# Dhole/collaborative_filtering

Measured on AMD Instinct MI355X. Metric: user-subgraph eigendecomps/sec + predicted ratings/sec, 1M users avg deg 100, higher is better.
Workload: dtype f32 (eigen) / f64 (predict)

## Files before the change

### collaborative_filtering_amd/_native.py

```python
from __future__ import annotations

import ctypes
import os
from ctypes import POINTER, c_char_p, c_double, c_float, c_int, c_int32, c_uint32, c_uint64, c_void_p

_HERE = os.path.dirname(os.path.abspath(__file__))
LIB_PATH = os.environ.get("CF_MI355X_LIB") or os.path.join(_HERE, "libcf_mi355x.so")
HOST_LIB_PATH = os.path.join(_HERE, "libcf_host.so")

CF_OK = 0
CF_EINVAL = -1
CF_ERANGE = -4
CF_ESTATE = -5
CF_KNN_SCORE_SUM = 0
CF_KNN_SCORE_MEAN = 1
CF_NMF_OBSERVED = 0
CF_NMF_GRID = 1
CF_NMF_EPS = 1e-16
CF_BPR_TRIES = 8
CF_SVD_MAX_NV = 256
CF_ALS_MAX_D = 64
CF_TOPN_MAX_N = 1024
CF_SIGS_OWN = 0
CF_SIGS_COMPAT = 1
CF_MAX_K = 192
CF_SPILL_MAX_K = 5000
CF_EIGEN_TRIDIAG = 0
CF_EIGEN_JACOBI = 1
CF_GRAPH_DENSE = 0
CF_GRAPH_CSR = 1
CF_FILTER_CHEBY = 0
CF_FILTER_BINOMIAL = 1

SIGNATURES = {
    "cf_version": (c_int, []),
    "cf_device_count": (c_int, []),
    "cf_create": (c_int, [c_int, POINTER(c_void_p)]),
    "cf_destroy": (None, [c_void_p]),
    "cf_release_workspaces": (c_int, [c_void_p]),
    "cf_last_error": (c_char_p, [c_void_p]),
    "cf_set_jacobi": (c_int, [c_void_p, c_float, c_int]),
    "cf_set_eigen_refine": (c_int, [c_void_p, c_int, c_float, c_float]),
    "cf_set_eigen_split": (c_int, [c_void_p, c_int]),
    "cf_set_eigen_lanes": (c_int, [c_void_p, c_int]),
    "cf_debug_eigen_geometry": (c_int, [c_int, c_int, POINTER(c_int), POINTER(c_int), POINTER(c_int), POINTER(c_int),
                                        POINTER(c_int)]),
    "cf_set_pred_pack": (c_int, [c_void_p, c_int]),
    "cf_debug_split_schedule": (c_int, [c_int, c_int, POINTER(c_int), POINTER(c_int), POINTER(c_int), POINTER(c_int)]),
    "cf_set_step_masks": (c_int, [c_void_p, c_int]),
    "cf_set_local_wlim": (c_int, [c_void_p, c_int]),
    "cf_debug_predict_nmax": (c_int, [c_int]),
    "cf_set_knn2_topk": (c_int, [c_void_p, c_uint32]),
    "cf_set_eigen_method": (c_int, [c_void_p, c_int]),
    "cf_debug_stats": (c_int, [c_void_p, c_int, c_void_p]),
    "cf_eigen_bucket_timing": (c_int, [c_void_p, c_int, c_void_p]),
    "cf_eigen_bucket_timing_split": (c_int, [c_void_p, c_int, c_void_p, c_void_p]),
    "cf_debug_phases": (c_int, [c_void_p, c_int, c_void_p]),
    "cf_debug_spill": (c_int, [c_void_p, c_int, c_void_p]),
    "cf_debug_tri": (c_int, [c_void_p, c_int, c_void_p]),
    "cf_item_graph_upload": (c_int, [c_void_p, c_uint32, c_void_p, c_void_p, c_void_p]),
    "cf_item_graph_upload_dense": (c_int, [c_void_p, c_uint32, c_void_p, c_int]),
    "cf_item_graph_device": (c_void_p, [c_void_p, POINTER(c_uint32)]),
    "cf_set_graph_layout": (c_int, [c_void_p, c_int]),
    "cf_graph_info": (c_int, [c_void_p, c_void_p, c_void_p, c_void_p]),
    "cf_item_cosine_edges": (c_int, [c_void_p, c_uint32, c_uint32, c_void_p, c_void_p, c_void_p, c_float, c_int, c_int,
                                     c_void_p, c_void_p, c_void_p, c_uint64, c_void_p]),
    "cf_plan_create": (c_int, [c_void_p, c_uint32, c_void_p, POINTER(c_void_p)]),
    "cf_plan_destroy": (None, [c_void_p]),
    "cf_evec_slots": (c_uint64, [c_uint32]),
    "cf_evec_offsets": (c_uint64, [c_uint32, c_void_p, c_void_p]),
    "cf_eigen_batch": (c_int, [c_void_p, c_uint32, c_void_p, c_void_p, c_void_p, c_void_p, c_void_p,
                               c_void_p, c_void_p]),
    "cf_eigen_run": (c_int, [c_void_p, c_void_p, c_void_p, c_void_p, c_void_p, c_void_p, c_void_p,
                             c_void_p, c_void_p, c_void_p]),
    "cf_predict_precomp": (c_int, [c_void_p, c_uint32, c_void_p, c_void_p, c_void_p, c_void_p, c_void_p,
                                   c_void_p, c_void_p, c_void_p, c_uint64, c_int, c_void_p, c_void_p,
                                   c_void_p]),
    "cf_predict_precomp_sel": (c_int, [c_void_p, c_uint32, c_void_p, c_void_p, c_void_p, c_void_p, c_void_p,
                                       c_void_p, c_void_p, c_void_p, c_uint64, c_int, c_void_p, c_void_p,
                                       c_void_p, c_void_p]),
# ... 238 lines not shown
```

### collaborative_filtering_amd/api.py

```python
from __future__ import annotations

from ctypes import byref, c_double, c_float, c_int, c_uint32, c_void_p
from dataclasses import dataclass

import numpy as np

from . import _native
from ._native import CF_ERANGE, CF_FILTER_BINOMIAL, CF_FILTER_CHEBY, CF_SIGS_COMPAT, CF_SIGS_OWN, NativeError, ptr


def _check(lib, ctx, rc, what):
    if rc != _native.CF_OK:
        msg = lib.cf_last_error(ctx)
        raise NativeError(f"{what} failed ({rc}): {msg.decode() if msg else ''}")


def evec_offsets(item_off: np.ndarray) -> tuple[np.ndarray, int]:
    k = np.diff(item_off.astype(np.int64))
    slots = k * np.maximum(k, 2)
    off = np.zeros(len(k), dtype=np.uint64)
    if len(k):
        off[1:] = np.cumsum(slots)[:-1]
    return off, int(slots.sum())

# ... 312 lines not shown
    def __enter__(self):
        return self

    def __exit__(self, *exc):
        self.close()

    def __del__(self):
        try:
            self.close()
        except Exception:
            pass

    def _chk(self, rc, what):
        _check(self.lib, self.h, rc, what)

    def set_eigen_method(self, method: str = "jacobi"):
        code = {"tridiag": _native.CF_EIGEN_TRIDIAG, "jacobi": _native.CF_EIGEN_JACOBI}[method]
        self._chk(self.lib.cf_set_eigen_method(self.h, code), "cf_set_eigen_method")

    def set_jacobi(self, tol_scale: float = 1.0, max_sweeps: int = 30):
        self._chk(self.lib.cf_set_jacobi(self.h, tol_scale, max_sweeps), "cf_set_jacobi")

    def set_eigen_refine(self, enable: bool = True, stop_rel: float = 1e-3, delta: float = 1e-2):
        self._chk(self.lib.cf_set_eigen_refine(self.h, int(enable), stop_rel, delta), "cf_set_eigen_refine")

    def set_eigen_split(self, enable=True):
        self._chk(self.lib.cf_set_eigen_split(self.h, int(enable)), "cf_set_eigen_split")

    def set_eigen_lanes(self, lanes=0):
        self._chk(self.lib.cf_set_eigen_lanes(self.h, int(lanes)), "cf_set_eigen_lanes")

    def set_pred_pack(self, mode=1):
        self._chk(self.lib.cf_set_pred_pack(self.h, int(mode)), "cf_set_pred_pack")

    def set_local_wlim(self, bisect: bool = True):
        self._chk(self.lib.cf_set_local_wlim(self.h, int(bisect)), "cf_set_local_wlim")

    def set_step_masks(self, enable: bool = True):
        self._chk(self.lib.cf_set_step_masks(self.h, int(enable)), "cf_set_step_masks")

    def debug_stats(self, enable: bool = True, read: bool = False):
        out = np.zeros(8, dtype=np.uint64) if read else None
        self._chk(self.lib.cf_debug_stats(self.h, int(enable), ptr(out)), "cf_debug_stats")
        if read:
            n = max(int(out[1]), 1)
            return {"sweeps_mean": int(out[0]) / n, "users": int(out[1]), "sweeps_max": int(out[2]),
                    "capped": int(out[3]), "assembly_cyc_per_user": int(out[4]) / n,
                    "jacobi_cyc_per_user": int(out[5]) / n, "epilogue_cyc_per_user": int(out[6]) / n,
                    "jacobi_cyc_per_step": int(out[5]) / max(int(out[7]), 1)}
        return None

    def eigen_bucket_timing(self, enable: bool = True, read: bool = False, sweeps: bool = False):
        out = np.zeros(13, dtype=np.float32) if read else None
        sw = np.zeros(13, dtype=np.float32) if read else None
        self._chk(self.lib.cf_eigen_bucket_timing_split(self.h, int(enable), ptr(out), ptr(sw)),
                  "cf_eigen_bucket_timing_split")
        return (out, sw) if sweeps else out

    def debug_spill(self, enable: bool = True, read: bool = False):
        out = np.zeros(8, dtype=np.uint64) if read else None
        self._chk(self.lib.cf_debug_spill(self.h, int(enable), ptr(out)), "cf_debug_spill")
        if read:
            n = max(int(out[0]), 1)
            names = ["assembly", "tridiag", "accumulate", "ql", "ql_gen"]
            r = {f"{nm}_cyc_per_user": int(out[i + 1]) / n for i, nm in enumerate(names)}
            r.update(users=int(out[0]), ql_iters_per_user=int(out[6]) / n, output_cyc_per_user=int(out[7]) / n)
# ... 962 lines not shown
```

### collaborative_filtering_amd/csrc/cf_internal.h

```cpp
#pragma once

#include <hip/hip_runtime.h>

#include <algorithm>
#include <cstdint>
#include <string>
#include <vector>

#include "cf_abi.h"

struct GraphRow {
    const float* dense;
    const uint32_t* col;
    const float* w;
    uint32_t len;
    __device__ __forceinline__ float operator[](uint32_t b) const {
        if (dense) return dense[b];
        uint32_t lo = 0, hi = len;
        while (lo < hi) {
            const uint32_t mid = (lo + hi) >> 1;
            if (col[mid] < b) lo = mid + 1;
            else hi = mid;
        }
        return (lo < len && col[lo] == b) ? w[lo] : 0.0f;
// ... 71 lines not shown
    size_t tri_bytes = 0;
    int eigen_method = CF_EIGEN_JACOBI;
    bool tri_debug = false;
    hipEvent_t knn_ev[3] = {nullptr, nullptr, nullptr};
    int knn_path = 0;
    unsigned int* d_knn_acc = nullptr;
    void* d_knn_part = nullptr;
    size_t knn_part_bytes = 0;
    uint32_t knn_chunk_users = 0;
    uint32_t knn2_topk = 0;
    int knn_chunks = 0;
    void* d_prep = nullptr;
    size_t prep_bytes = 0;
    hipEvent_t prep_ev[2] = {nullptr, nullptr};
    static constexpr int kAuxStreams = 2;
    hipStream_t aux_stream[kAuxStreams] = {};
    hipEvent_t aux_event[kAuxStreams + 1] = {};
    static constexpr int kBucketRuns = 16;
    bool bucket_timing = false;
    hipEvent_t bucket_ev[kBucketRuns][13][3] = {};
    bool bucket_recorded[kBucketRuns][13] = {};
    bool bucket_mid[kBucketRuns][13] = {};
    hipEvent_t split_mid_ev = nullptr;
    bool split_mid_recorded = false;
    int bucket_run = 0;
    hipStream_t step_stream[2] = {};
    hipEvent_t step_bucket_ev[16] = {};
    hipEvent_t step_sync_ev[4] = {};
    hipEvent_t step_time_ev[3] = {};
    uint32_t* d_split_sched[13] = {};
    int eigen_lanes = -1;
    int eigen_split = -1;
    int pred_pack = -1;
    int split_finish = -1;
    float filter_ms = 0.0f;
    uint64_t filter_nnz = 0;
    void* d_als = nullptr;
    size_t als_bytes = 0;
    float sgd_reduce_ms[2] = {0.0f, 0.0f};
    float svdpp_reduce_ms[3] = {0.0f, 0.0f, 0.0f};
    float bpr_ms[6] = {0.0f, 0.0f, 0.0f, 0.0f, 0.0f, 0.0f};
    uint32_t topn_block = 0;
    uint64_t* d_knn_in_off = nullptr;
    uint32_t* d_knn_in_m = nullptr;
    float* d_knn_in_w = nullptr;
    uint32_t* d_knn_in_cnt = nullptr;
    double knn_in_wmin = 0.0;
    uint64_t knn_in_gen = ~0ull;
    int knn_topn_wgs = -1;
    double* d_ease_B = nullptr;
    uint32_t ease_n = 0;
    float ease_ms[3] = {0.0f, 0.0f, 0.0f};
};

void cf_ease_free(cf_ctx* ctx);

void cf_knn_in_free(cf_ctx* ctx);

struct PanelSource {
    virtual ~PanelSource() = default;
    virtual bool valid() const = 0;
    virtual size_t workspace(uint32_t ub) const = 0;
    virtual int upload(cf_ctx* ctx, void* ws, uint32_t ub, hipStream_t st, float* score_ms) = 0;
    virtual int fill(cf_ctx* ctx, hipStream_t st, const uint32_t* d_sel, uint32_t b0, uint32_t nb, uint64_t* d_panel) = 0;
};
int cf_topn_drive(cf_ctx* ctx, const char* fn, PanelSource& src, uint32_t n_users, uint32_t n_items,
// ... 209 lines not shown
```

### collaborative_filtering_amd/csrc/cf_predict.hip

```cpp
#include "cf_internal.h"
#include "cf_ldlt.hpp"

namespace {

constexpr int kThreads = 256;
constexpr int kWaves = kThreads / 64;
constexpr int kNsysMax = 62;
constexpr int kQuadNMax = 14;
constexpr int kPairNMax = 30;
constexpr int fast_tri(int n) { return (n + 2) * (n + 3) / 2; }
constexpr int pack_elems(int G, int nG, int lmax) { return G * (fast_tri(nG) + lmax + nG); }
constexpr double kPivMin = 1e-10;
constexpr double kOrthoMax = 1e-2;
constexpr float kOrthoDone = 1e-8f;
#ifndef CF_PRED_FS_PW
#define CF_PRED_FS_PW 8
#endif
constexpr int kFsPw = CF_PRED_FS_PW;
#ifndef CF_PRED_BASIS_OCC
#define CF_PRED_BASIS_OCC 3
#endif

struct SlotOff {
    size_t stride;
    int gb, x, q1, ap, gx, hx, misc, cmask, lim, order, cpos, pmask;
};

template <typename T>
struct PredArgs {
    const uint32_t* order;
    const uint64_t* item_off;
    const uint32_t* items;
    const float* ratings;
    const uint8_t* row_sel;
    const int32_t* m;
    const T* evals;
    const uint64_t* evec_off;
    const T* evecs;
    const T* sigtab;
    int sig_mode;
    GraphDev graph;
    uint64_t n_items;
    float* mse;
    int32_t* kk;
    double* pred;
    unsigned long long* phase_cycles;
    int lmax;
    int nmax;
    int ew;
    int pack;
    int a_elems;
    int big_lds;
    int tail_basis;
    const uint64_t* cmask_in;
    uint64_t cmask_words;
    const uint64_t* cmask_fp;
    uint32_t cmask_users;
    double* slots;
    SlotOff so;
    uint32_t* dq;
    double* dense_ws;
};


template <int CTRL>
__device__ __forceinline__ double dpp_f64(double v) {
    const int lo = __builtin_amdgcn_update_dpp(0, __double2loint(v), CTRL, 0xf, 0xf, false);
    const int hi = __builtin_amdgcn_update_dpp(0, __double2hiint(v), CTRL, 0xf, 0xf, false);
    return __hiloint2double(hi, lo);
}
__device__ __forceinline__ double row16_sum(double v) {
    v += dpp_f64<0xB1>(v);
    v += dpp_f64<0x4E>(v);
    v += dpp_f64<0x141>(v);
    v += dpp_f64<0x140>(v);
    return v;
}
__device__ __forceinline__ double lane_f64(double v, int l) {
    return __hiloint2double(__builtin_amdgcn_readlane(__double2hiint(v), l), __builtin_amdgcn_readlane(__double2loint(v), l));
}
#ifdef CF_PRED_SHFL_SUM
__device__ __forceinline__ double wave_sum(double v) {
#pragma unroll
// ... 13 lines not shown
#else
    double x = __builtin_amdgcn_rcp(d);
    double e = fma(-d, x, 1.0);
    x = fma(x, e, x);
    e = fma(-d, x, 1.0);
    return fma(x, e, x);
#endif
}

__device__ int block_compact(bool flag, int idx, int* out, int* s_cnt) {
    const int tid = threadIdx.x;
    const int lane = tid & 63;
    const int wave = tid >> 6;
    const unsigned long long bal = __ballot(flag);
    if (lane == 0) s_cnt[wave] = __popcll(bal);
    __syncthreads();
    int off = 0;
    for (int w = 0; w < wave; ++w) off += s_cnt[w];
    if (flag) out[off + __popcll(bal & ((1ull << lane) - 1ull))] = idx;
    const int total = s_cnt[0] + s_cnt[1] + s_cnt[2] + s_cnt[3];
    __syncthreads();
    return total;
}

constexpr int kStageLd = 80;
constexpr int kStageBuf = 2 * 16 * kStageLd;
#ifdef CF_PRED_GEMM_SINGLE_BUFFER
constexpr int kStageNbuf = 1;
#else
constexpr int kStageNbuf = 2;
#endif
constexpr int kStageElems = kStageNbuf * kStageBuf;
using f64x4 = __attribute__((ext_vector_type(4))) double;
template <bool A_LFAST, bool B_LFAST, bool LOWER = false, class LA, class XA, class LB, class XB, class FK, class FW,
          class FO>
__device__ void block_gemm(int M, int N, LA loadA, XA xA, LB loadB, XB xB, FK kend, FW want, FO out,
                           double* stage) {
    int tid = threadIdx.x;
    __asm__ volatile("" : "+v"(tid));
    const int lane = tid & 63;
    const int wr = (tid >> 6) >> 1, wc = (tid >> 6) & 1;
    using RA = decltype(loadA(0, 0));
    using RB = decltype(loadB(0, 0));
    for (int i0 = 0; i0 < M; i0 += 64)
        for (int j0 = 0; j0 < N; j0 += 64) {
            if (!want(i0, j0)) continue;
            const int K = kend(j0);
            bool live[2][2];
#pragma unroll
            for (int x = 0; x < 2; ++x)
#pragma unroll
                for (int y = 0; y < 2; ++y) {
                    const int ti = i0 + 32 * wr + 16 * x, tj = j0 + 32 * wc + 16 * y;
#ifdef CF_PRED_GEMM_NOSKIP
                    live[x][y] = ti == ti && tj == tj;
#else
                    live[x][y] = ti < M && tj < N && (!LOWER || tj <= ti + 15);
#endif
                }
            f64x4 acc[2][2];
#pragma unroll
            for (int x = 0; x < 2; ++x)
#pragma unroll
                for (int y = 0; y < 2; ++y) acc[x][y] = f64x4{0.0, 0.0, 0.0, 0.0};
            RA ra0[4], ra1[4];
            RB rb0[4], rb1[4];
            auto fetch = [&](int l0, RA (&ra)[4], RB (&rb)[4]) {
#pragma unroll
                for (int t = 0; t < 4; ++t) {
                    const int e = tid + kThreads * t;
                    const int ia = A_LFAST ? (e >> 4) : (e & 63), la = A_LFAST ? (e & 15) : (e >> 6);
                    const int jb = B_LFAST ? (e >> 4) : (e & 63), lb = B_LFAST ? (e & 15) : (e >> 6);
                    ra[t] = loadA(min(i0 + ia, M - 1), min(l0 + la, K - 1));
                    rb[t] = loadB(min(l0 + lb, K - 1), min(j0 + jb, N - 1));
                }
            };
            auto stage_chunk = [&](int l0, RA (&ra)[4], RB (&rb)[4], int b) {
                double* As = stage + (kStageNbuf - 1) * b * kStageBuf;
                double* Bs = As + 16 * kStageLd;
                if (kStageNbuf == 1) __syncthreads();
#pragma unroll
                for (int t = 0; t < 4; ++t) {
                    const int e = tid + kThreads * t;
                    const int ia = A_LFAST ? (e >> 4) : (e & 63), la = A_LFAST ? (e & 15) : (e >> 6);
                    const int jb = B_LFAST ? (e >> 4) : (e & 63), lb = B_LFAST ? (e & 15) : (e >> 6);
                    const bool oka = i0 + ia < M && l0 + la < K;
                    const bool okb = j0 + jb < N && l0 + lb < K;
                    As[la * kStageLd + ia] = oka ? xA(i0 + ia, l0 + la, ra[t]) : 0.0;
                    Bs[lb * kStageLd + jb] = okb ? xB(l0 + lb, j0 + jb, rb[t]) : 0.0;
                }
                __syncthreads();
            };
            auto mma_chunk = [&](int b) {
                const double* As = stage + (kStageNbuf - 1) * b * kStageBuf;
                const double* Bs = As + 16 * kStageLd;
#pragma unroll
                for (int ks = 0; ks < 4; ++ks) {
                    const int row = (4 * ks + (lane >> 4)) * kStageLd + (lane & 15);
                    double av[2], bv[2];
#pragma unroll
                    for (int x = 0; x < 2; ++x) {
                        av[x] = As[row + 32 * wr + 16 * x];
                        bv[x] = Bs[row + 32 * wc + 16 * x];
                    }
#pragma unroll
                    for (int x = 0; x < 2; ++x)
#pragma unroll
                        for (int y = 0; y < 2; ++y)
                            if (live[x][y])
                                acc[x][y] = __builtin_amdgcn_mfma_f64_16x16x4f64(av[x], bv[y], acc[x][y], 0, 0, 0);
                }
            };
            if (K > 0) fetch(0, ra0, rb0);
            if (K > 16) fetch(16, ra1, rb1);
            for (int l0 = 0; l0 < K; l0 += 32) {
                stage_chunk(l0, ra0, rb0, 0);
                if (l0 + 32 < K) fetch(l0 + 32, ra0, rb0);
                mma_chunk(0);
                if (l0 + 16 < K) {
                    stage_chunk(l0 + 16, ra1, rb1, 1);
                    if (l0 + 48 < K) fetch(l0 + 48, ra1, rb1);
                    mma_chunk(1);
                }
            }
            if (kStageNbuf == 2) __syncthreads();
#pragma unroll
            for (int x = 0; x < 2; ++x)
#pragma unroll
                for (int y = 0; y < 2; ++y)
#pragma unroll
                    for (int q = 0; q < 4; ++q) {
                        const int i = i0 + 32 * wr + 16 * x + (lane >> 4) + 4 * q;
                        const int j = j0 + 32 * wc + 16 * y + (lane & 15);
                        if (i < M && j < N) out(i, j, acc[x][y][q]);
                    }
        }
}

template <int NS, int PF, class LOAD>
__device__ void wave_gram_t(int nt, int inner, LOAD load, double* E) {
    constexpr int NT = NS * (NS + 1) / 2;
    const int lane = threadIdx.x & 63;
    const int li = lane & 15, lk = lane >> 4;
    f64x4 acc[NT];
#pragma unroll
    for (int x = 0; x < NT; ++x) acc[x] = f64x4{0.0, 0.0, 0.0, 0.0};
    double v[PF][NS], w[PF][NS];
    auto fetch = [&](int s0) {
#pragma unroll
        for (int p = 0; p < PF; ++p)
#pragma unroll
            for (int t = 0; t < NS; ++t) w[p][t] = load(16 * t + li, s0 + 4 * p + lk);
    };
    fetch(0);
    for (int s0 = 0; s0 < inner; s0 += 4 * PF) {
#pragma unroll
        for (int p = 0; p < PF; ++p)
#pragma unroll
            for (int t = 0; t < NS; ++t) v[p][t] = w[p][t];
        if (s0 + 4 * PF < inner) fetch(s0 + 4 * PF);
#pragma unroll
        for (int p = 0; p < PF; ++p) {
            if (s0 + 4 * p >= inner) break;
            int x = 0;
#pragma unroll
            for (int ti = 0; ti < NS; ++ti)
#pragma unroll
// ... 138 lines not shown
                }
                if (lane == 0 && r0 + x < k) s_slow[r0 + x] = nc;
            }
        }
        __syncthreads();
        for (int i = tid; i < k; i += kThreads) {
            const int ni = s_slow[i];
            int rank = 0;
            for (int j = 0; j < k; ++j) {
                const int nj = s_slow[j];
                rank += (nj > ni) || (nj == ni && j < i);
            }
            s_order[rank] = i;
        }

        double* stage = A;
        if (tid == 0) s_cnt[6] = 0;
        __syncthreads();
        unsigned long long tg0 = (a.phase_cycles && tid == 0) ? __builtin_amdgcn_s_memtime() : 0ull;
        const auto all_blocks = [](int, int) { return true; };
        const auto lower_blocks = [](int i0, int j0) { return j0 <= i0; };
        float dev = 0.0f;
        const auto as_double = [](int, int, auto v) { return (double)v; };
        const auto tri_T = [](int l, int j, double g) { return l < j ? -g : (l == j ? 1.5 - 0.5 * g : 0.0); };
        block_gemm<false, false, true>(
            Lu, Lu, [&](int i, int l) { return U[(size_t)l * m + i]; }, as_double,
            [&](int l, int j) { return U[(size_t)l * m + j]; }, as_double, [&](int) { return k; }, lower_blocks,
            [&](int i, int j, double v) {
                if (j > i) return;
                Gb[(size_t)j * lmax + i] = v;
                const float d = (float)fabs(v - (i == j ? 1.0 : 0.0));
                dev = fmaxf(dev, d == d ? d : 3.0e38f);
            },
            stage);
        for (int off = 32; off >= 1; off >>= 1) dev = fmaxf(dev, __shfl_xor(dev, off));
        if (lane == 0) atomicMax(&s_cnt[6], __float_as_int(dev));
        __syncthreads();
#ifndef CF_PRED_BASIS_PROBE
        if (a.phase_cycles && tid == 0) ph_acc[6] += __builtin_amdgcn_s_memtime() - tg0;
#endif
        {
            uint64_t* pm_g = reinterpret_cast<uint64_t*>(slot + a.so.pmask);
            for (int j = tid; j < Lu; j += kThreads) {
                int cnt = 0, sole = 0;
#pragma unroll
                for (int w = 0; w < 3; ++w) {
                    uint64_t bits = 0;
                    const int iend = min(k, 64 * w + 64);
                    for (int i0 = 64 * w; i0 < iend; i0 += 16) {
                        double v[16];
#pragma unroll
                        for (int t = 0; t < 16; ++t) v[t] = (double)U[(size_t)min(i0 + t, k - 1) * m + j];
#pragma unroll
                        for (int t = 0; t < 16; ++t)
                            if (i0 + t < iend && v[t] >= 0.0001) bits |= 1ull << (i0 + t - 64 * w);
                    }
                    pm_g[3 * j + w] = bits;
                    cnt += __popcll(bits);
                    if (bits) sole = 64 * w + __builtin_ctzll(bits);
                }
                s_cpos[j] = cnt;
                if (cnt == 0) atomicMin(&s_cnt[11], j);
                if (cnt == 1) atomicMin(&s_dmin[sole], j);
            }
        }
        __syncthreads();
        const int Lq = (__int_as_float(s_cnt[6]) <= (float)kOrthoMax) ? Lu : 0;
        PHASE_STAMP(0);

        double* Q1 = slot + a.so.q1;
        double* Xb = slot + a.so.x;
        double* AP = slot + a.so.ap;
        const int ld = lmax;
        double* Xf = Xb;
        int Lx = 0;
        int jlo = 0;
        if (Lq > 0) {
            if (tid == 0) s_cnt[9] = 0;
            const auto tri_end = [&](int j0) { return min(Lq, j0 + 64); };
            block_gemm<true, false>(
                k, Lq, [&](int i, int l) { return U[(size_t)i * m + l]; }, as_double,
                [&](int l, int j) { return Gb[(size_t)l * lmax + j]; }, tri_T, tri_end, all_blocks,
                [&](int i, int j, double v) { Xb[(size_t)i * ld + j] = v; }, stage);
            __syncthreads();
#ifdef CF_PRED_BASIS_PROBE
            const unsigned long long tw0 = (a.phase_cycles && tid == 0) ? __builtin_amdgcn_s_memtime() : 0ull;
#endif
            const int du = k - Lq;
            if (du > 0) {
                const auto mix = [](uint32_t h) {
                    h ^= h >> 16;
                    h *= 0x7FEB352Du;
                    h ^= h >> 15;
                    h *= 0x846CA68Bu;
                    return h ^ (h >> 16);
                };
                const uint32_t seed = mix(mix(mix((uint32_t)k * 0x9E3779B1u + 0x7F4A7C15u) ^ s_item[0]) ^
                                          s_item[k >> 1]) ^ s_item[k - 1];
                const auto omega = [seed](int i, int j) -> double {
                    uint32_t h = seed ^ ((uint32_t)i * 0x85EBCA6Bu) ^ ((uint32_t)j * 0xC2B2AE35u);
                    h ^= h >> 16;
                    h *= 0x7FEB352Du;
                    h ^= h >> 15;
                    h *= 0x846CA68Bu;
                    h ^= h >> 16;
                    return (h & 1u) ? 1.0 : -1.0;
                };
                const auto om = [&](int l, int j) { return omega(l, j); };
                block_gemm<false, false>(
                    Lq, du, [&](int i, int l) { return Xb[(size_t)l * ld + i]; }, as_double, om, as_double,
                    [&](int) { return k; }, all_blocks, [&](int i, int j, double v) { Q1[(size_t)i * ld + j] = v; },
                    stage);
                __syncthreads();
                block_gemm<true, false>(
                    k, du, [&](int i, int l) { return Xb[(size_t)i * ld + l]; }, as_double,
                    [&](int l, int j) { return Q1[(size_t)l * ld + j]; }, as_double, [&](int) { return Lq; },
                    all_blocks, [&](int i, int j, double v) { Xb[(size_t)i * ld + Lq + j] = omega(i, j) - v; }, stage);
                __syncthreads();
                block_gemm<false, false, true>(
                    du, du, [&](int i, int l) { return Xb[(size_t)l * ld + Lq + i]; }, as_double,
                    [&](int l, int j) { return Xb[(size_t)l * ld + Lq + j]; }, as_double, [&](int) { return k; },
                    lower_blocks, [&](int i, int j, double v) { if (j <= i) AP[tri(i, j)] = v; }, stage);
                __syncthreads();
                double* LP = AP;
#ifndef CF_PRED_COMPLEMENT_GLOBAL
                if (tri(du, 0) <= kStageElems) {
                    LP = stage;
                    for (int i = tid; i < tri(du, 0); i += kThreads) LP[i] = AP[i];
                    __syncthreads();
                }
#endif
                ldlt_bordered<kThreads, 16>(LP, du, du);
                double dmax = 0.0;
                for (int j = 0; j < du; ++j) dmax = fmax(dmax, LP[tri(j, j)]);
                bool fail = false;
                for (int i = tid; i < k; i += kThreads) {
                    double* xi = Xb + (size_t)i * ld + Lq;
                    for (int p0 = 0; p0 < du; p0 += kFsPw) {
                        const int b = min(kFsPw, du - p0);
                        double acc[kFsPw];
                        int rb[kFsPw];
#pragma unroll
                        for (int q = 0; q < kFsPw; ++q) {
                            acc[q] = q < b ? xi[p0 + q] : 0.0;
                            rb[q] = tri(p0 + min(q, b - 1), 0);
                        }
#pragma unroll 2
                        for (int t = 0; t < p0; ++t) {
                            const double xt = xi[t];
#pragma unroll
                            for (int q = 0; q < kFsPw; ++q) acc[q] = fma(-LP[rb[q] + t], xt, acc[q]);
                        }
#pragma unroll
                        for (int q = 1; q < kFsPw; ++q)
#pragma unroll
// ... 4 lines not shown
                    }
                    for (int j = 0; j < du; ++j) {
                        const double dj = LP[tri(j, j)];
                        fail |= !(dj > 1e-12 * dmax);
                        xi[j] = dj > 0.0 ? xi[j] / sqrt(dj) : 0.0;
                    }
                }
                if (fail) s_cnt[9] = 1;
                __syncthreads();
            }
#ifdef CF_PRED_BASIS_PROBE
            if (a.phase_cycles && tid == 0) ph_acc[7] += __builtin_amdgcn_s_memtime() - tw0;
            const unsigned long long tj0 = (a.phase_cycles && tid == 0) ? __builtin_amdgcn_s_memtime() : 0ull;
#endif
            double* Xs = Xb;
            double* Xd = Q1;
            jlo = a.tail_basis ? (min(s_cnt[10], k) & ~63) : 0;
            if (s_cnt[9] == 0) {
                for (int it = 0; it < 3; ++it) {
                    if (tid == 0) s_cnt[6] = 0;
                    __syncthreads();
                    float dv = 0.0f;
                    const int glo = jlo;
                    block_gemm<false, false, true>(
                        k, k, [&](int i, int l) { return Xs[(size_t)l * ld + i]; }, as_double,
                        [&](int l, int j) { return Xs[(size_t)l * ld + j]; }, as_double, [&](int) { return k; },
                        [glo](int i0, int j0) { return j0 <= i0 && (i0 >= glo || i0 == j0); },
                        [&](int i, int j, double v) {
                            if (j > i) return;
                            AP[tri(i, j)] = v;
                            const float dd = (float)fabs(v - (i == j ? 1.0 : 0.0));
                            dv = fmaxf(dv, dd == dd ? dd : 3.0e38f);
                        },
                        stage);
                    for (int off = 32; off >= 1; off >>= 1) dv = fmaxf(dv, __shfl_xor(dv, off));
                    if (lane == 0) atomicMax(&s_cnt[6], __float_as_int(dv));
                    __syncthreads();
                    const float dev_x = __int_as_float(s_cnt[6]);
                    if (!(dev_x <= (float)kOrthoMax)) break;
                    if (glo > 0 && !(dev_x <= kOrthoDone)) {
                        jlo = 0;
                        --it;
                        __syncthreads();
                        continue;
                    }
                    const auto k_end = [&](int j0) { return min(k, j0 + 64); };
                    block_gemm<true, false>(
                        k, k, [&](int i, int l) { return Xs[(size_t)i * ld + l]; }, as_double,
                        [&](int l, int j) { return AP[tri(max(l, j), min(l, j))]; }, tri_T, k_end,
                        [glo](int, int j0) { return j0 >= glo; },
                        [&](int i, int j, double v) { Xd[(size_t)i * ld + j] = v; }, stage);
                    __syncthreads();
                    double* tmp = Xs;
                    Xs = Xd;
                    Xd = tmp;
                    if (dev_x <= kOrthoDone) {
                        Lx = k;
                        break;
                    }
                }
            }
            Xf = Xs;
#ifdef CF_PRED_BASIS_PROBE
            if (a.phase_cycles && tid == 0) ph_acc[6] += __builtin_amdgcn_s_memtime() - tj0;
#endif
        }
        double* s_gx = slot + a.so.gx;
        double* s_hx = slot + a.so.hx;
        double* gxl = A;
        double* hxl = A + CF_MAX_K;
        int* s_list = reinterpret_cast<int*>(A + 2 * CF_MAX_K);
        if (Lx > 0)
            for (int j = jlo + tid; j < k; j += kThreads) {
                double g0 = 0.0, g1 = 0.0, h0 = 0.0, h1 = 0.0;
                int i = 0;
                for (; i + 1 < k; i += 2) {
                    const double x0 = Xf[(size_t)i * ld + j], x1 = Xf[(size_t)(i + 1) * ld + j];
                    g0 = fma(x0, (double)s_rat[i], g0);
                    g1 = fma(x1, (double)s_rat[i + 1], g1);
                    h0 += x0;
                    h1 += x1;
                }
                if (i < k) {
                    const double x0 = Xf[(size_t)i * ld + j];
                    g0 = fma(x0, (double)s_rat[i], g0);
                    h0 += x0;
                }
                s_gx[j] = gxl[j] = g0 + g1;
                s_hx[j] = hxl[j] = h0 + h1;
            }
        __syncthreads();
        int n_rate = k;
#ifdef CF_PRED_NO_CLOSED
        if (false) {
#else
        if (Lx > 0 && m >= 2 && k >= 2) {
#endif
            const int zmin = s_cnt[11];
            const bool cand = tid < k && s_slow[tid] == 1 && ((s_cmask[3 * tid + (tid >> 6)] >> (tid & 63)) & 1ull) &&
                              s_lim[tid] < k && s_lim[tid] <= zmin && s_lim[tid] <= s_dmin[tid];
            const int ncand = block_compact(cand, tid, s_list, s_cnt);
            const double sum_all = s_misc[1];
            const int gl = tid & 15;
            for (int e = tid >> 4; e < ncand; e += kThreads / 16) {
                const int r = s_list[e];
                const int lim = s_lim[r];
                const int d = k - lim;
                const double rr = (double)s_rat[r];
                const double mu = (sum_all - rr) / (double)(k - 1);
                double kq = 0.0, bg = 0.0;
                for (int j = gl; j < d; j += 16) {
                    const double x = Xf[(size_t)r * ld + lim + j];
                    const double g = gxl[lim + j] - mu * hxl[lim + j];
                    kq = fma(x, x, kq);
                    bg = fma(x, g, bg);
                }
                kq = row16_sum(kq);
                bg = row16_sum(bg);
// ... 961 lines not shown
        if (chunk <= 256) return cf_set_error(ctx, CF_ENOMEM, "predictor slots (" + std::to_string(need) + " bytes)");
        chunk /= 2;
    }
}
inline size_t basis_lds() {
    return sizeof(double) * (kStageElems + 4) + CF_MAX_K * (sizeof(uint32_t) + sizeof(float) + 3 * sizeof(int)) +
           12 * sizeof(int) + CF_MAX_K * (3 * sizeof(uint64_t) + 2 * sizeof(int));
}
static_assert(2 * CF_MAX_K + CF_MAX_K / 2 <= kStageElems, "closed-form LDS copies exceed the staging area");
inline size_t rating_lds_fixed() {
    return sizeof(double) * (4 + 2 * CF_MAX_K) +
           CF_MAX_K * (sizeof(uint32_t) + sizeof(float) + 6 * sizeof(int)) + 12 * sizeof(int) +
           CF_MAX_K * (3 * sizeof(uint64_t) + sizeof(int)) + kWaves * CF_MAX_K * sizeof(int) +
           3 * CF_MAX_K * sizeof(uint64_t);
}

template <typename T>
int setup_bucket(cf_ctx* ctx, PredArgs<T>& args, int lmax, size_t& rating_lds) {
    args.lmax = lmax;
    const size_t lds_fixed = rating_lds_fixed();
    const int big = (lmax + 2) * (lmax + 3) / 2;
    const auto per_wave = [&](int n) { return fast_tri(n) + 2 * lmax; };
    int nmax = std::min(kNsysMax, lmax);
    while (nmax > 8 && sizeof(double) * (size_t)(kWaves * per_wave(nmax)) + lds_fixed > kRatingLds) --nmax;
    args.nmax = nmax;
    args.ew = per_wave(nmax);
    if (ctx->pred_pack < 0) {
        const char* e = std::getenv("CF_PRED_PACK");
        ctx->pred_pack = e && e[0] == '0' ? 0 : 1;
    }
    const int ew_pack = std::max(pack_elems(4, kQuadNMax, lmax), pack_elems(2, kPairNMax, lmax));
    args.pack = ctx->pred_pack && sizeof(double) * (size_t)(kWaves * std::max(args.ew, ew_pack)) + lds_fixed <= kRatingLds;
    if (args.pack) args.ew = std::max(args.ew, ew_pack);
    args.big_lds = sizeof(double) * (size_t)std::max(big, kWaves * args.ew) + lds_fixed <= kRatingLds;
    args.a_elems = std::max({args.big_lds ? big : 0, kWaves * args.ew, 2 * lmax});
    args.so = slot_layout(lmax);
    rating_lds = sizeof(double) * (size_t)args.a_elems + lds_fixed;
    if (rating_lds > 163840) return cf_set_error(ctx, CF_ERANGE, "predict bucket exceeds LDS");
    CF_HIP_CHECK(ctx, hipFuncSetAttribute((const void*)pred_dense_kernel<T>, hipFuncAttributeMaxDynamicSharedMemorySize,
                                          (int)rating_lds));
    CF_HIP_CHECK(ctx, hipFuncSetAttribute((const void*)pred_rating_kernel<T>,
                                          hipFuncAttributeMaxDynamicSharedMemorySize, (int)rating_lds));
    CF_HIP_CHECK(ctx, hipFuncSetAttribute((const void*)pred_basis_kernel<T>,
                                          hipFuncAttributeMaxDynamicSharedMemorySize, (int)basis_lds()));
    return CF_OK;
}

inline bool pred_fused_enabled() {
    static const bool on = [] {
        const char* e = std::getenv("CF_PRED_FUSED");
        return e && e[0] == '1';
    }();
    return on;
}

inline int pred_tail_basis() {
    static const int on = [] {
        const char* e = std::getenv("CF_PRED_TAIL");
        return e && e[0] == '0' ? 0 : 1;
    }();
    return on;
}

template <typename T>
int fused_geometry(cf_ctx* ctx, size_t rating_lds, uint32_t grid_cap, uint32_t& grid, size_t& lds) {
    lds = std::max(rating_lds, basis_lds());
// ... 325 lines not shown
    return static_cast<uint64_t*>(ctx->d_cmask);
}

void cf_cmask_mark(cf_ctx* ctx, const cf_plan* plan, const uint64_t* d_item_off, const uint32_t* d_items, bool valid) {
    ctx->cmask_plan = plan->id;
    ctx->cmask_key[0] = d_item_off;
    ctx->cmask_key[1] = d_items;
    ctx->cmask_gen = valid ? ctx->graph_gen : ~0ull;
}

const uint64_t* cf_cmask_lookup(const cf_ctx* ctx, const cf_plan* plan, const uint64_t* d_item_off,
                                const uint32_t* d_items) {
    const bool hit = ctx->d_cmask && ctx->cmask_gen == ctx->graph_gen && ctx->cmask_plan == plan->id &&
                     ctx->cmask_key[0] == d_item_off && ctx->cmask_key[1] == d_items;
    return hit ? static_cast<const uint64_t*>(ctx->d_cmask) : nullptr;
}

template int cf_launch_predict<float>(cf_ctx*, const cf_plan*, const uint64_t*, const uint32_t*,
                                      const float*, const int32_t*, const float*, const uint64_t*,
                                      const float*, const float*, int, float*, int32_t*, double*,
                                      const uint8_t*, hipStream_t);
template int cf_launch_predict<double>(cf_ctx*, const cf_plan*, const uint64_t*, const uint32_t*,
                                       const float*, const int32_t*, const double*,
                                       const uint64_t*, const double*, const double*, int, float*,
                                       int32_t*, double*, const uint8_t*, hipStream_t);

extern "C" int cf_set_pred_pack(cf_ctx* ctx, int mode) {
    if (!ctx) return CF_EINVAL;
    if (mode != 0 && mode != 1) return CF_EINVAL;
    ctx->pred_pack = mode;
    return CF_OK;
}

extern "C" int cf_debug_predict_nmax(int lmax) {
    if (lmax < 2 || lmax > CF_MAX_K) return -1;
    const size_t lds_fixed = rating_lds_fixed();
    const auto per_wave = [&](int n) { return fast_tri(n) + 2 * lmax; };
    int nmax = std::min(kNsysMax, lmax);
    while (nmax > 8 && sizeof(double) * (size_t)(kWaves * per_wave(nmax)) + lds_fixed > kRatingLds) --nmax;
    return nmax;
}
```

### include/cf_abi.h

```cpp
#ifndef CF_ABI_H
#define CF_ABI_H

#include <stddef.h>
#include <stdint.h>

#ifdef __cplusplus
extern "C" {
#endif

#define CF_OK 0
#define CF_EINVAL (-1)
#define CF_ENOMEM (-2)
#define CF_EHIP (-3)
#define CF_ERANGE (-4)
#define CF_ESTATE (-5)

#define CF_MAX_K 192
#define CF_SPILL_MAX_K 5000

typedef struct cf_ctx cf_ctx;
typedef struct cf_plan cf_plan;

int cf_version(void);
int cf_device_count(void);
int cf_create(int device, cf_ctx** out);
void cf_destroy(cf_ctx* ctx);
int cf_release_workspaces(cf_ctx* ctx);
const char* cf_last_error(const cf_ctx* ctx);
#define CF_EIGEN_TRIDIAG 0
#define CF_EIGEN_JACOBI 1
int cf_set_eigen_method(cf_ctx* ctx, int method);
int cf_set_jacobi(cf_ctx* ctx, float tol_scale, int max_sweeps);
int cf_set_eigen_refine(cf_ctx* ctx, int enable, float stop_rel, float delta);
int cf_set_eigen_split(cf_ctx* ctx, int enable);
int cf_set_eigen_lanes(cf_ctx* ctx, int lanes);
int cf_debug_eigen_geometry(int emax, int lanes_setting, int* lanes, int* threads, int* ld, int* lds_bytes,
                            int* users_per_cu);
int cf_set_pred_pack(cf_ctx* ctx, int mode);
int cf_debug_split_schedule(int emax, int k, int* steps, int* levels, int* max_groups, int* max_slots);
int cf_set_step_masks(cf_ctx* ctx, int enable);
int cf_set_local_wlim(cf_ctx* ctx, int bisect);
int cf_debug_stats(cf_ctx* ctx, int enable, uint64_t* out8);
int cf_debug_spill(cf_ctx* ctx, int enable, uint64_t* out8);
int cf_debug_tri(cf_ctx* ctx, int enable, uint64_t* out8);
int cf_debug_phases(cf_ctx* ctx, int enable, uint64_t* out16);
int cf_debug_predict_nmax(int lmax);
int cf_eigen_bucket_timing(cf_ctx* ctx, int enable, float* ms13);
int cf_eigen_bucket_timing_split(cf_ctx* ctx, int enable, float* ms13, float* sweeps_ms13);

#define CF_GRAPH_DENSE 0
#define CF_GRAPH_CSR 1
int cf_set_graph_layout(cf_ctx* ctx, int layout);
int cf_graph_info(const cf_ctx* ctx, int* layout, uint32_t* n_items, uint64_t* nnz);
int cf_item_graph_upload(cf_ctx* ctx, uint32_t n_items, const uint64_t* row_ptr,
                         const uint32_t* col, const float* w);
int cf_item_graph_upload_dense(cf_ctx* ctx, uint32_t n_items, const float* w_dense,
                               int on_device);
const float* cf_item_graph_device(const cf_ctx* ctx, uint32_t* n_items);

int cf_plan_create(cf_ctx* ctx, uint32_t n_users, const uint64_t* item_off, cf_plan** out);
void cf_plan_destroy(cf_plan* plan);
uint64_t cf_evec_slots(uint32_t k);
uint64_t cf_evec_offsets(uint32_t n_users, const uint64_t* item_off, uint64_t* evec_off);

int cf_eigen_batch(cf_ctx* ctx, uint32_t n_users, const uint64_t* item_off,
                   const uint32_t* items, const uint64_t* evec_off, int32_t* m_out,
                   float* sigs, float* evals, float* evecs);
int cf_eigen_run(cf_ctx* ctx, const cf_plan* plan, const uint64_t* d_item_off,
                 const uint32_t* d_items, const uint64_t* d_evec_off, int32_t* d_m,
                 float* d_sigs, float* d_evals, float* d_evecs, void* stream);

// ... 357 lines not shown
```

Measured before the change: 312,600.

## Deal live 16x16 GEMM tiles evenly across waves and deepen X^T r loads

Replaces the fixed 2x2 wave-to-quadrant mapping in the prediction block GEMM with a table-driven assignment. Live 16x16 sub-tiles of partial or lower-triangular 64x64 blocks are spread across the four waves, with an optional per-block rotation so that edge blocks do not leave waves idle. Separately, the X^T-rating reduction loop now batches several rows of loads ahead of the FMAs to expose more memory-level parallelism. Both raise register use and add a constant-memory lookup per block, and the deal mode is on by default behind an env/API toggle.

```diff
diff --git a/collaborative_filtering_amd/_native.py b/collaborative_filtering_amd/_native.py
--- a/collaborative_filtering_amd/_native.py
+++ b/collaborative_filtering_amd/_native.py
@@ -46,6 +46,9 @@
     "cf_debug_eigen_geometry": (c_int, [c_int, c_int, POINTER(c_int), POINTER(c_int), POINTER(c_int), POINTER(c_int),
                                         POINTER(c_int)]),
     "cf_set_pred_pack": (c_int, [c_void_p, c_int]),
+    "cf_set_pred_gemm_deal": (c_int, [c_void_p, c_int]),
+    "cf_debug_pred_gemm_deal": (c_int, [c_int, c_int, c_int, c_int, POINTER(c_int), POINTER(c_int), POINTER(c_int),
+                                        POINTER(c_int), POINTER(c_int)]),
     "cf_debug_split_schedule": (c_int, [c_int, c_int, POINTER(c_int), POINTER(c_int), POINTER(c_int), POINTER(c_int)]),
     "cf_set_step_masks": (c_int, [c_void_p, c_int]),
     "cf_set_local_wlim": (c_int, [c_void_p, c_int]),
diff --git a/collaborative_filtering_amd/api.py b/collaborative_filtering_amd/api.py
--- a/collaborative_filtering_amd/api.py
+++ b/collaborative_filtering_amd/api.py
@@ -368,6 +368,9 @@
 
     def set_pred_pack(self, mode=1):
         self._chk(self.lib.cf_set_pred_pack(self.h, int(mode)), "cf_set_pred_pack")
+
+    def set_pred_gemm_deal(self, mode=1):
+        self._chk(self.lib.cf_set_pred_gemm_deal(self.h, int(mode)), "cf_set_pred_gemm_deal")
 
     def set_local_wlim(self, bisect: bool = True):
         self._chk(self.lib.cf_set_local_wlim(self.h, int(bisect)), "cf_set_local_wlim")
diff --git a/collaborative_filtering_amd/csrc/cf_internal.h b/collaborative_filtering_amd/csrc/cf_internal.h
--- a/collaborative_filtering_amd/csrc/cf_internal.h
+++ b/collaborative_filtering_amd/csrc/cf_internal.h
@@ -127,6 +127,7 @@
     int eigen_lanes = -1;
     int eigen_split = -1;
     int pred_pack = -1;
+    int pred_gemm_deal = -1;
     int split_finish = -1;
     float filter_ms = 0.0f;
     uint64_t filter_nnz = 0;
diff --git a/collaborative_filtering_amd/csrc/cf_pred_gemm_deal.h b/collaborative_filtering_amd/csrc/cf_pred_gemm_deal.h
--- /dev/null
+++ b/collaborative_filtering_amd/csrc/cf_pred_gemm_deal.h
@@ -0,0 +1,17 @@
+#define CF_PRED_GEMM_DEAL_TABLE \
+    0x144, 0x0e4, 0x04e, 0x0ee, 0x344, 0x0e4, 0x04e, 0x0ee, 0x344, 0x1e4, 0x04e, 0x0ee, 0x344, 0x3e4, 0x04e, 0x0ee, \
+    0x544, 0x0e4, 0x04e, 0x0ee, 0xf44, 0x0e4, 0x04e, 0x0ee, 0xf44, 0x5e4, 0x04e, 0x0ee, 0xf44, 0xfe4, 0x04e, 0x0ee, \
+    0x544, 0x0e4, 0x14e, 0x0ee, 0xf44, 0x0e4, 0x34e, 0x0ee, 0xf44, 0x5e4, 0x34e, 0x1ee, 0xf44, 0xfe4, 0x34e, 0x3ee, \
+    0x544, 0x0e4, 0x54e, 0x0ee, 0xf44, 0x0e4, 0xf4e, 0x0ee, 0xf44, 0x5e4, 0xf4e, 0x5ee, 0xf44, 0xfe4, 0xf4e, 0xfee, \
+    0x144, 0x0e4, 0x04e, 0x0ee, 0x144, 0x0e4, 0x04e, 0x0ee, 0x144, 0x0e4, 0x04e, 0x0ee, 0x144, 0x0e4, 0x04e, 0x0ee, \
+    0x544, 0x0e4, 0x04e, 0x0ee, 0xd44, 0x0e4, 0x04e, 0x0ee, 0xd44, 0x0e4, 0x04e, 0x0ee, 0xd44, 0x0e4, 0x04e, 0x0ee, \
+    0x544, 0x0e4, 0x14e, 0x0ee, 0xd44, 0x0e4, 0x34e, 0x0ee, 0xd44, 0x0e4, 0x34e, 0x1ee, 0xd44, 0x0e4, 0x34e, 0x1ee, \
+    0x544, 0x0e4, 0x54e, 0x0ee, 0xd44, 0x0e4, 0xf4e, 0x0ee, 0xd44, 0x0e4, 0xf4e, 0x5ee, 0xd44, 0x0e4, 0xf4e, 0xdee, \
+    0x100, 0x000, 0x000, 0x000, 0x100, 0x150, 0x000, 0x000, 0x100, 0x150, 0x1a0, 0x000, 0x100, 0x150, 0x1a0, 0x1f0, \
+    0x100, 0x105, 0x000, 0x000, 0x100, 0x150, 0x105, 0x155, 0x340, 0x684, 0x395, 0x000, 0x340, 0x3e0, 0x345, 0x3e5, \
+    0x100, 0x105, 0x10a, 0x000, 0x340, 0x345, 0x34a, 0x000, 0x744, 0xe94, 0x34a, 0x1aa, 0x744, 0x7e4, 0xe49, 0xee9, \
+    0x100, 0x105, 0x10a, 0x10f, 0x340, 0x345, 0x34a, 0x34f, 0x744, 0xe94, 0x74e, 0xe9e, 0xf44, 0xfe4, 0xf4e, 0xfee, \
+    0x100, 0x000, 0x000, 0x000, 0x100, 0x000, 0x000, 0x000, 0x100, 0x000, 0x000, 0x000, 0x100, 0x000, 0x000, 0x000, \
+    0x100, 0x105, 0x000, 0x000, 0x100, 0x105, 0x155, 0x000, 0x100, 0x105, 0x155, 0x000, 0x100, 0x105, 0x155, 0x000, \
+    0x100, 0x105, 0x10a, 0x000, 0x504, 0x649, 0x15a, 0x000, 0x504, 0x649, 0x39a, 0x000, 0x504, 0x649, 0x39a, 0x000, \
+    0x100, 0x105, 0x10a, 0x10f, 0x504, 0x649, 0x64e, 0x15f, 0xd44, 0x74e, 0xe9e, 0x000, 0xd44, 0x74e, 0xe9e, 0x1ff
diff --git a/collaborative_filtering_amd/csrc/cf_predict.hip b/collaborative_filtering_amd/csrc/cf_predict.hip
--- a/collaborative_filtering_amd/csrc/cf_predict.hip
+++ b/collaborative_filtering_amd/csrc/cf_predict.hip
@@ -1,4 +1,5 @@
 #include "cf_internal.h"
+#include "cf_pred_gemm_deal.h"
 #include "cf_ldlt.hpp"
 
 namespace {
@@ -17,6 +18,10 @@
 #define CF_PRED_FS_PW 8
 #endif
 constexpr int kFsPw = CF_PRED_FS_PW;
+#ifndef CF_PRED_XTR_DEPTH
+#define CF_PRED_XTR_DEPTH 8
+#endif
+constexpr int kXtrDepth = CF_PRED_XTR_DEPTH;
 #ifndef CF_PRED_BASIS_OCC
 #define CF_PRED_BASIS_OCC 3
 #endif
@@ -49,6 +54,7 @@
     int nmax;
     int ew;
     int pack;
+    int gemm_deal;
     int a_elems;
     int big_lds;
     int tail_basis;
@@ -128,32 +134,36 @@
 #endif
 constexpr int kStageElems = kStageNbuf * kStageBuf;
 using f64x4 = __attribute__((ext_vector_type(4))) double;
+__constant__ uint32_t kGemmDealDev[2 * 2 * 4 * 4 * 4] = {CF_PRED_GEMM_DEAL_TABLE};
+const uint32_t kGemmDealHost[2 * 2 * 4 * 4 * 4] = {CF_PRED_GEMM_DEAL_TABLE};
 template <bool A_LFAST, bool B_LFAST, bool LOWER = false, class LA, class XA, class LB, class XB, class FK, class FW,
           class FO>
 __device__ void block_gemm(int M, int N, LA loadA, XA xA, LB loadB, XB xB, FK kend, FW want, FO out,
-                           double* stage) {
+                           double* stage, int deal) {
     int tid = threadIdx.x;
     __asm__ volatile("" : "+v"(tid));
     const int lane = tid & 63;
-    const int wr = (tid >> 6) >> 1, wc = (tid >> 6) & 1;
+    const int wave = __builtin_amdgcn_readfirstlane(tid >> 6);
+    int turn = 0;
     using RA = decltype(loadA(0, 0));
     using RB = decltype(loadB(0, 0));
     for (int i0 = 0; i0 < M; i0 += 64)
         for (int j0 = 0; j0 < N; j0 += 64) {
             if (!want(i0, j0)) continue;
             const int K = kend(j0);
+#ifdef CF_PRED_GEMM_NOSKIP
+            const int rl = 4, cl = 4, dg = 0;
+#else
+            const int rl = min(4, (M - i0 + 15) >> 4), cl = min(4, (N - j0 + 15) >> 4), dg = LOWER && i0 == j0;
+#endif
+            const uint32_t pe = kGemmDealDev[((((deal * 2 + dg) * 4 + rl - 1) * 4 + cl - 1) << 2) + ((wave + turn) & 3)];
+            turn += deal;
+            const int tr[2] = {(int)(pe & 3u), (int)(pe >> 2 & 3u)}, tc[2] = {(int)(pe >> 4 & 3u), (int)(pe >> 6 & 3u)};
             bool live[2][2];
 #pragma unroll
             for (int x = 0; x < 2; ++x)
 #pragma unroll
-                for (int y = 0; y < 2; ++y) {
-                    const int ti = i0 + 32 * wr + 16 * x, tj = j0 + 32 * wc + 16 * y;
-#ifdef CF_PRED_GEMM_NOSKIP
-                    live[x][y] = ti == ti && tj == tj;
-#else
-                    live[x][y] = ti < M && tj < N && (!LOWER || tj <= ti + 15);
-#endif
-                }
+                for (int y = 0; y < 2; ++y) live[x][y] = pe >> (8 + 2 * x + y) & 1u;
             f64x4 acc[2][2];
 #pragma unroll
             for (int x = 0; x < 2; ++x)
@@ -196,8 +206,8 @@
                     double av[2], bv[2];
 #pragma unroll
                     for (int x = 0; x < 2; ++x) {
-                        av[x] = As[row + 32 * wr + 16 * x];
-                        bv[x] = Bs[row + 32 * wc + 16 * x];
+                        av[x] = As[row + 16 * tr[x]];
+                        bv[x] = Bs[row + 16 * tc[x]];
                     }
 #pragma unroll
                     for (int x = 0; x < 2; ++x)
@@ -226,9 +236,9 @@
                 for (int y = 0; y < 2; ++y)
 #pragma unroll
                     for (int q = 0; q < 4; ++q) {
-                        const int i = i0 + 32 * wr + 16 * x + (lane >> 4) + 4 * q;
-                        const int j = j0 + 32 * wc + 16 * y + (lane & 15);
-                        if (i < M && j < N) out(i, j, acc[x][y][q]);
+                        const int i = i0 + 16 * tr[x] + (lane >> 4) + 4 * q;
+                        const int j = j0 + 16 * tc[y] + (lane & 15);
+                        if (live[x][y] && i < M && j < N) out(i, j, acc[x][y][q]);
                     }
         }
 }
@@ -433,7 +443,7 @@
                 const float d = (float)fabs(v - (i == j ? 1.0 : 0.0));
                 dev = fmaxf(dev, d == d ? d : 3.0e38f);
             },
-            stage);
+            stage, a.gemm_deal);
         for (int off = 32; off >= 1; off >>= 1) dev = fmaxf(dev, __shfl_xor(dev, off));
         if (lane == 0) atomicMax(&s_cnt[6], __float_as_int(dev));
         __syncthreads();
@@ -482,7 +492,7 @@
             block_gemm<true, false>(
                 k, Lq, [&](int i, int l) { return U[(size_t)i * m + l]; }, as_double,
                 [&](int l, int j) { return Gb[(size_t)l * lmax + j]; }, tri_T, tri_end, all_blocks,
-                [&](int i, int j, double v) { Xb[(size_t)i * ld + j] = v; }, stage);
+                [&](int i, int j, double v) { Xb[(size_t)i * ld + j] = v; }, stage, a.gemm_deal);
             __syncthreads();
 #ifdef CF_PRED_BASIS_PROBE
             const unsigned long long tw0 = (a.phase_cycles && tid == 0) ? __builtin_amdgcn_s_memtime() : 0ull;
@@ -511,17 +521,17 @@
                 block_gemm<false, false>(
                     Lq, du, [&](int i, int l) { return Xb[(size_t)l * ld + i]; }, as_double, om, as_double,
                     [&](int) { return k; }, all_blocks, [&](int i, int j, double v) { Q1[(size_t)i * ld + j] = v; },
-                    stage);
+                    stage, a.gemm_deal);
                 __syncthreads();
                 block_gemm<true, false>(
                     k, du, [&](int i, int l) { return Xb[(size_t)i * ld + l]; }, as_double,
                     [&](int l, int j) { return Q1[(size_t)l * ld + j]; }, as_double, [&](int) { return Lq; },
-                    all_blocks, [&](int i, int j, double v) { Xb[(size_t)i * ld + Lq + j] = omega(i, j) - v; }, stage);
+                    all_blocks, [&](int i, int j, double v) { Xb[(size_t)i * ld + Lq + j] = omega(i, j) - v; }, stage, a.gemm_deal);
                 __syncthreads();
                 block_gemm<false, false, true>(
                     du, du, [&](int i, int l) { return Xb[(size_t)l * ld + Lq + i]; }, as_double,
                     [&](int l, int j) { return Xb[(size_t)l * ld + Lq + j]; }, as_double, [&](int) { return k; },
-                    lower_blocks, [&](int i, int j, double v) { if (j <= i) AP[tri(i, j)] = v; }, stage);
+                    lower_blocks, [&](int i, int j, double v) { if (j <= i) AP[tri(i, j)] = v; }, stage, a.gemm_deal);
                 __syncthreads();
                 double* LP = AP;
 #ifndef CF_PRED_COMPLEMENT_GLOBAL
@@ -592,7 +602,7 @@
                             const float dd = (float)fabs(v - (i == j ? 1.0 : 0.0));
                             dv = fmaxf(dv, dd == dd ? dd : 3.0e38f);
                         },
-                        stage);
+                        stage, a.gemm_deal);
                     for (int off = 32; off >= 1; off >>= 1) dv = fmaxf(dv, __shfl_xor(dv, off));
                     if (lane == 0) atomicMax(&s_cnt[6], __float_as_int(dv));
                     __syncthreads();
@@ -609,7 +619,7 @@
                         k, k, [&](int i, int l) { return Xs[(size_t)i * ld + l]; }, as_double,
                         [&](int l, int j) { return AP[tri(max(l, j), min(l, j))]; }, tri_T, k_end,
                         [glo](int, int j0) { return j0 >= glo; },
-                        [&](int i, int j, double v) { Xd[(size_t)i * ld + j] = v; }, stage);
+                        [&](int i, int j, double v) { Xd[(size_t)i * ld + j] = v; }, stage, a.gemm_deal);
                     __syncthreads();
                     double* tmp = Xs;
                     Xs = Xd;
@@ -633,17 +643,32 @@
         if (Lx > 0)
             for (int j = jlo + tid; j < k; j += kThreads) {
                 double g0 = 0.0, g1 = 0.0, h0 = 0.0, h1 = 0.0;
-                int i = 0;
-                for (; i + 1 < k; i += 2) {
-                    const double x0 = Xf[(size_t)i * ld + j], x1 = Xf[(size_t)(i + 1) * ld + j];
-                    g0 = fma(x0, (double)s_rat[i], g0);
-                    g1 = fma(x1, (double)s_rat[i + 1], g1);
-                    h0 += x0;
-                    h1 += x1;
-                }
-                if (i < k) {
-                    const double x0 = Xf[(size_t)i * ld + j];
-                    g0 = fma(x0, (double)s_rat[i], g0);
+                const int kp = k & ~1;
+                int kpv = kp;
+                __asm__ volatile("" : "+v"(kpv));
+                for (int i = 0; i < kp; i += 2 * kXtrDepth) {
+                    double x0[kXtrDepth], x1[kXtrDepth];
+                    float r0[kXtrDepth], r1[kXtrDepth];
+#pragma unroll
+                    for (int t = 0; t < kXtrDepth; ++t) {
+                        const int r = min(i + 2 * t, kp - 2);
+                        x0[t] = Xf[(size_t)r * ld + j];
+                        x1[t] = Xf[(size_t)(r + 1) * ld + j];
+                        r0[t] = s_rat[r];
+                        r1[t] = s_rat[r + 1];
+                    }
+#pragma unroll
+                    for (int t = 0; t < kXtrDepth; ++t) {
+                        const bool in = kXtrDepth == 1 || i + 2 * t < kpv;
+                        g0 = in ? fma(x0[t], (double)r0[t], g0) : g0;
+                        g1 = in ? fma(x1[t], (double)r1[t], g1) : g1;
+                        h0 = in ? h0 + x0[t] : h0;
+                        h1 = in ? h1 + x1[t] : h1;
+                    }
+                }
+                if (kp < k) {
+                    const double x0 = Xf[(size_t)kp * ld + j];
+                    g0 = fma(x0, (double)s_rat[kp], g0);
                     h0 += x0;
                 }
                 s_gx[j] = gxl[j] = g0 + g1;
@@ -1671,6 +1696,11 @@
     const int ew_pack = std::max(pack_elems(4, kQuadNMax, lmax), pack_elems(2, kPairNMax, lmax));
     args.pack = ctx->pred_pack && sizeof(double) * (size_t)(kWaves * std::max(args.ew, ew_pack)) + lds_fixed <= kRatingLds;
     if (args.pack) args.ew = std::max(args.ew, ew_pack);
+    if (ctx->pred_gemm_deal < 0) {
+        const char* e = std::getenv("CF_PRED_GEMM_DEAL");
+        ctx->pred_gemm_deal = e && e[0] == '0' ? 0 : 1;
+    }
+    args.gemm_deal = ctx->pred_gemm_deal;
     args.big_lds = sizeof(double) * (size_t)std::max(big, kWaves * args.ew) + lds_fixed <= kRatingLds;
     args.a_elems = std::max({args.big_lds ? big : 0, kWaves * args.ew, 2 * lmax});
     args.so = slot_layout(lmax);
@@ -2062,6 +2092,29 @@
     return CF_OK;
 }
 
+extern "C" int cf_set_pred_gemm_deal(cf_ctx* ctx, int mode) {
+    if (!ctx) return CF_EINVAL;
+    if (mode != 0 && mode != 1) return CF_EINVAL;
+    ctx->pred_gemm_deal = mode;
+    return CF_OK;
+}
+
+extern "C" int cf_debug_pred_gemm_deal(int deal, int rows_live, int cols_live, int diag, int* r0, int* r1, int* c0,
+                                       int* c1, int* mask) {
+    if ((deal != 0 && deal != 1) || (diag != 0 && diag != 1) || rows_live < 1 || rows_live > 4 || cols_live < 1 ||
+        cols_live > 4)
+        return CF_EINVAL;
+    for (int w = 0; w < kWaves; ++w) {
+        const uint32_t pe = kGemmDealHost[((((deal * 2 + diag) * 4 + rows_live - 1) * 4 + cols_live - 1) << 2) + w];
+        if (r0) r0[w] = pe & 3u;
+        if (r1) r1[w] = pe >> 2 & 3u;
+        if (c0) c0[w] = pe >> 4 & 3u;
+        if (c1) c1[w] = pe >> 6 & 3u;
+        if (mask) mask[w] = pe >> 8 & 15u;
+    }
+    return CF_OK;
+}
+
 extern "C" int cf_debug_predict_nmax(int lmax) {
     if (lmax < 2 || lmax > CF_MAX_K) return -1;
     const size_t lds_fixed = rating_lds_fixed();
diff --git a/include/cf_abi.h b/include/cf_abi.h
--- a/include/cf_abi.h
+++ b/include/cf_abi.h
@@ -37,6 +37,9 @@
 int cf_debug_eigen_geometry(int emax, int lanes_setting, int* lanes, int* threads, int* ld, int* lds_bytes,
                             int* users_per_cu);
 int cf_set_pred_pack(cf_ctx* ctx, int mode);
+int cf_set_pred_gemm_deal(cf_ctx* ctx, int mode);
+int cf_debug_pred_gemm_deal(int deal, int rows_live, int cols_live, int diag, int* r0, int* r1, int* c0, int* c1,
+                            int* mask);
 int cf_debug_split_schedule(int emax, int k, int* steps, int* levels, int* max_groups, int* max_slots);
 int cf_set_step_masks(cf_ctx* ctx, int enable);
 int cf_set_local_wlim(cf_ctx* ctx, int bisect);
```

After: 315,500, median of 6. Within noise of the previous version (+0.9%).
